# salute-developers/GigaAM

Hardware: AMD Instinct MI355X
Metric: RTFx v2_ctc batch32x20s (log-mel + encoder + greedy decode) (higher is better)
Workload: dtype f32 (GEMMs: 3-term split on fp16 MFMA, fp32 accumulate)

## Files before the change

### gigaam_amd/_lib.py

```python
from __future__ import annotations

import ctypes as C
import os
from typing import Optional

_HERE = os.path.dirname(os.path.abspath(__file__))
LIB_NAME = "libgigaam_hip.so"
LIB_PATH = os.path.join(_HERE, LIB_NAME)

SUBS_CONV2D, SUBS_CONV1D = 0, 1
ATT_ROTARY, ATT_REL_POS = 0, 1
NORM_BATCH, NORM_LAYER = 0, 1
HEAD_NONE, HEAD_CTC, HEAD_RNNT, HEAD_EMO = 0, 1, 2, 3
DTYPE_F32, DTYPE_F16, DTYPE_BF16, DTYPE_F64, DTYPE_I64 = 0, 1, 2, 3, 4
GEMM_F32, GEMM_F16X3, GEMM_F16 = 0, 1, 2
RS_U8, RS_I16, RS_I24, RS_I32, RS_F32, RS_MULAW, RS_ALAW = range(7)
RS_FORM_SINGLE, RS_FORM_TABLE, RS_FORM_ROWS = 0, 1, 2
PF_CLASSES = ["gemm", "conv2", "attn", "norm", "convmod", "stem", "frontend", "decode", "misc", "align_bt", "align_out"]


class GamConfig(C.Structure):
    _fields_ = [(n, C.c_int32) for n in (
        "sample_rate", "n_mels", "hop_length", "win_length", "n_fft", "center",
        "feat_in", "n_layers", "d_model", "subsampling", "subs_kernel_size", "subsampling_factor",
# ... 66 lines not shown
    "gam_op_ctc_confidence": (C.c_int, [_P, _P, _P, C.c_int, C.c_int64, C.c_int, _P, _P, _P, C.c_int, C.c_int, C.c_int, _P, _P, _P, _P]),
    "gam_op_ctc_confidence_long": (C.c_int, [_P, _P, C.c_int64, C.c_int, _P, _P, _P, C.c_int, C.c_int, C.c_int, C.c_int, _P, _P, _P, _P]),
    "gam_rnnt_confidence": (C.c_int, [_P, _P, _P, C.c_int, C.c_int64, _P, _P, _P, C.c_int, C.c_int, _P, _P, _P]),
    "gam_op_rnnt_confidence": (C.c_int, [_P, _P, _P, C.c_int, C.c_int64, _P, _P, _P, C.c_int, C.c_int, _P, _P, _P]),
    "gam_emo_probs": (C.c_int, [_P, _P, _P, C.c_int, C.c_int64, _P, _P]),
    "gam_rnnt_predict": (C.c_int, [_P, _P, _P, _P, C.c_int, _P, _P, _P, _P]),
    "gam_rnnt_joint": (C.c_int, [_P, _P, _P, C.c_int, C.c_int, C.c_int, _P, _P]),
    "gam_set_gemm_mode": (C.c_int, [_P, C.c_int]),
    "gam_get_gemm_mode": (C.c_int, [_P]),
    "gam_set_rnnt_cluster": (C.c_int, [_P, C.c_int]),
    "gam_get_rnnt_cluster": (C.c_int, [_P]),
    "gam_rnnt_cluster_plan_info": (C.c_int, [C.c_int] * 8 + [C.POINTER(C.c_int32)]),
    "gam_rnnt_last_decode": (C.c_int, [_P, C.POINTER(C.c_int32)]),
    "gam_debug_buffer_hash": (C.c_int, [_P, C.c_int, C.POINTER(C.c_uint64), C.POINTER(C.c_int64)]),
    "gam_range_flag": (C.c_int, [_P, C.POINTER(C.c_int), _P]),
    "gam_range_flag_fetch": (C.c_int, [_P, _P, _P]),
    "gam_op_gemm": (C.c_int, [_P, _P, _P, _P, _P, C.c_int, C.c_int, C.c_int, C.c_int, _P]),
    "gam_op_gemm_ex": (C.c_int, [_P, _P, _P, _P, _P, C.c_float, _P, C.c_int, C.c_int, C.c_int, C.c_int, _P]),
    "gam_op_attention": (C.c_int, [_P, _P, _P, _P, _P, _P, C.c_int, C.c_int, C.c_int, _P]),
    "gam_op_attention_ex": (C.c_int, [_P, _P, _P, _P, C.c_int64, _P, _P, _P, C.c_int, C.c_int, C.c_int, C.c_int, _P, _P, _P, _P]),
    "gam_op_layernorm": (C.c_int, [_P, C.POINTER(GamLnOp), _P]),
    "gam_op_convmod": (C.c_int, [_P, _P, _P, _P, _P, _P, _P, _P, _P, C.c_int, C.c_int, C.c_int, C.c_int, C.c_int, C.c_int, C.c_int, _P]),
    "gam_tune_sp": (C.c_int, [C.c_int, C.c_int, C.c_int]),
    "gam_plan_sp": (C.c_int, [C.c_int, C.c_int, C.c_int, C.c_int, C.POINTER(C.c_int), C.POINTER(C.c_int), C.POINTER(C.c_int)]),
    "gam_plan_sp_ex": (C.c_int, [C.c_int, C.c_int, C.c_int, C.c_int, C.POINTER(C.c_int), C.POINTER(C.c_int), C.POINTER(C.c_int), C.POINTER(C.c_int)]),
    "gam_tune_sp_stages": (C.c_int, [C.c_int]),
    "gam_resample_plan": (C.c_int, [C.c_int, C.c_int, C.POINTER(C.c_int), C.POINTER(C.c_int), C.POINTER(C.c_int)]),
    "gam_resample_tile": (C.c_int, [C.c_int, C.c_int, C.POINTER(C.c_int), C.POINTER(C.c_int)]),
    "gam_resample_table": (C.c_int, [C.c_int, C.c_int, _P, _P]),
    "gam_resample_out_len": (C.c_int64, [C.c_int, C.c_int, C.c_int64]),
    "gam_op_resample": (C.c_int, [_P, C.c_int, C.c_int, C.c_int, _P, C.c_int, C.c_int64, C.c_int, C.c_int, _P, _P, _P, C.c_int64, _P, _P]),
    "gam_profile_enable": (C.c_int, [_P, C.c_int]),
    "gam_profile_pause": (C.c_int, [_P, C.c_int]),
    "gam_profile_read": (C.c_int, [_P, C.c_int, C.POINTER(C.c_double), C.POINTER(C.c_int64), C.POINTER(C.c_double)]),
    "gam_profile_read_bytes": (C.c_int, [_P, C.c_int, C.POINTER(C.c_double)]),
    "gam_last_error": (C.c_char_p, [_P]),
    "gam_comm_unique_id": (C.c_int, [C.c_char_p]),
    "gam_comm_create": (C.c_int, [C.c_char_p, C.c_int, C.c_int, C.c_int, C.POINTER(_P)]),
    "gam_comm_world": (C.c_int, [_P]),
    "gam_gather_ids": (C.c_int, [_P, _P, _P, _P, _P, C.c_int, C.c_int, _P, _P, _P, _P, _P]),
    "gam_comm_last_error": (C.c_char_p, [_P]),
    "gam_comm_destroy": (None, [_P]),
}

_lib: Optional[C.CDLL] = None

# ... 25 lines not shown
```

### gigaam_amd/csrc/gam_api.hip

```cpp
#include <hip/hip_runtime.h>

#include <algorithm>
#include <cmath>
#include <cstdarg>
#include <cstdio>
#include <cstring>
#include <map>
#include <string>
#include <vector>

#include "../../include/gigaam_hip.h"
#include "gam_align.h"
#include "gam_align_long.h"
#include "gam_kws.h"
#include "gam_attn.h"
#include "gam_beam.h"
#include "gam_beam_stream.h"
#include "gam_rnnt_beam.h"
#include "gam_attn16.h"
#include "gam_comm.h"
#include "gam_common.h"
#include "gam_convmod.h"
#include "gam_decode.h"
#include "gam_rnnt_align.h"
// ... 410 lines not shown

GamGemmArgs gemm_args(const float* A, long lda, const float* W, const float* bias, float* C, long ldc, int M, int N, int K) {
  GamGemmArgs g;
  memset(&g, 0, sizeof g);
  g.A = A; g.W = W; g.bias = bias; g.C = C; g.R = nullptr;
  g.M = M; g.N = N; g.K = K; g.lda = lda; g.ldc = ldc; g.ldr = ldc; g.alpha = 1.0f;
  g.rpb = 1; g.fdiv = 1;
  return g;
}

int layernorm(gam_handle* h, hipStream_t s, GamLnArgs a, int mode, PendingReduce* pend = nullptr) {
  if (pend != nullptr && pend->part != nullptr) {
    const GamGemmArgs& g = pend->full;
    if (a.x == g.C && a.rows == g.M && a.d == g.N && g.ldc == g.N) {
      a.part = pend->part; a.nsplit = pend->nsplit; a.pbias = pend->bias; a.presid = pend->resid; a.palpha = pend->alpha;
      a.xstore = const_cast<float*>(a.x);
      pend->clear();
    } else if (int r = flush_pending(h, s, pend)) {
      return r;
    }
  }
  const double bytes = (double)a.rows * a.d * 4.0 * (mode == 0 ? 2.0 : 3.0);
  ProfScope ps(h, s, GAM_PF_NORM, bytes);
  hipError_t e = gam_launch_layernorm(a, mode, s);
  if (e != hipSuccess) return fail(h, -2, "layernorm launch: %s", hipGetErrorString(e));
  return 0;
}

int64_t half_up(int64_t l) { return l <= 0 ? 0 : (l + 1) / 2; }

struct DecodeScope {
  gam_handle* h;
  hipStream_t s;
  DecodeScope(gam_handle* h_, hipStream_t s_) : h(h_), s(s_) {
    if (h->dec_evt == nullptr && hipEventCreateWithFlags(&h->dec_evt, hipEventDisableTiming) != hipSuccess) { h->dec_evt = nullptr; (void)hipGetLastError(); }
    if (h->dec_evt != nullptr && h->dec_evt_set && h->dec_stream != s) (void)hipStreamWaitEvent(s, h->dec_evt, 0);
  }
  ~DecodeScope() {
    if (h->dec_evt != nullptr && hipEventRecord(h->dec_evt, s) == hipSuccess) { h->dec_stream = s; h->dec_evt_set = true; }
  }
};

#define GAM_DECODE_ENTRY(h, stream)      \
  hipStream_t s = (hipStream_t)(stream); \
  if (!(h)) return -1;                   \
  HIPCHK(h, hipSetDevice((h)->device));  \
  DecodeScope ds(h, s)
// ... 2252 lines not shown
    return fail(h, -1, "layernorm: store format %d / %d outside 0..2", o.split1, o.split2);
  if (!o.out1 || !o.w1 || !o.b1) return fail(h, -1, "layernorm: out1 / w1 / b1 are mandatory");
  if (!o.part && !o.x) return fail(h, -1, "layernorm: x is mandatory without part");
  if (o.part && o.mode != 2 && !o.xstore) return fail(h, -1, "layernorm: part without xstore");
  if (o.mode != 0 && !o.out2) return fail(h, -1, "layernorm: mode %d needs out2", o.mode);
  if (o.mode == 2 && (!o.w2 || !o.b2)) return fail(h, -1, "layernorm: mode 2 needs w2 / b2");
  if (o.mode == 1) {
    if (!o.rcos || !o.rsin || o.rope_rows <= 0) return fail(h, -1, "layernorm: mode 1 needs rcos / rsin of rope_rows > 0 rows");
    if (o.dk <= 0) return fail(h, -1, "layernorm: mode 1 needs dk > 0");
    if (!o.row_t && o.ta <= 0) return fail(h, -1, "layernorm: mode 1 needs row_t or ta > 0");
  }
  auto al16 = [](const void* p) { return (reinterpret_cast<uintptr_t>(p) & 15) == 0; };
  if (!al16(o.x) || !al16(o.out1) || !al16(o.out2) || !al16(o.w1) || !al16(o.b1) || !al16(o.w2) || !al16(o.b2) || !al16(o.rcos) ||
      !al16(o.rsin) || !al16(o.part) || !al16(o.pbias) || !al16(o.presid) || !al16(o.xstore))
    return fail(h, -1, "layernorm: operands must be 16-byte aligned");
  HIPCHK(h, hipSetDevice(h->device));
  GamLnArgs a;
  memset(&a, 0, sizeof a);
  a.x = o.x; a.out1 = o.out1; a.out2 = o.out2; a.w1 = o.w1; a.b1 = o.b1; a.w2 = o.w2; a.b2 = o.b2;
  a.rcos = o.rcos; a.rsin = o.rsin; a.rows = o.rows; a.d = o.d; a.ta = o.ta; a.dk = o.dk; a.eps = o.eps;
  a.split1 = o.split1; a.split2 = o.split2; a.rs = o.rs; a.rope_rows = o.rope_rows;
  a.part = o.part; a.nsplit = o.nsplit; a.pbias = o.pbias; a.presid = o.presid; a.palpha = o.palpha; a.xstore = o.xstore;
  a.row_t = o.row_t;
  hipError_t e = gam_launch_layernorm(a, o.mode, (hipStream_t)stream);
  if (e != hipSuccess)
    return fail(h, -2, "layernorm launch (mode %d, rows %d, d %d, dk %d, split %d/%d, nsplit %d): %s", o.mode, o.rows, o.d, o.dk,
                o.split1, o.split2, o.part ? o.nsplit : 0, hipGetErrorString(e));
  return 0;
}

int gam_op_convmod(gam_handle* h, const float* u, float* z, const float* dw_w, const float* dw_b, const float* n_scale,
                   const float* n_shift, const int32_t* lens, const int32_t* cu, int B, int Ta, int Tv, int d, int ks, int layer_norm,
                   int z_split, void* stream) {
  if (!h) return -1;
  if (!h->finalized) return fail(h, -1, "gam_op_convmod before gam_finalize");
  if (!u || !z || !dw_w || !dw_b || !n_scale || !n_shift || !lens) return fail(h, -1, "conv module: null operand");
  if (B <= 0 || Ta <= 0 || Tv <= 0 || d <= 0) return fail(h, -1, "conv module: bad shape B %d Ta %d Tv %d d %d", B, Ta, Tv, d);
  if (cu == nullptr && Tv > Ta) return fail(h, -1, "conv module: Tv %d > Ta %d in the padded layout", Tv, Ta);
  if (z_split < 0 || z_split > 2) return fail(h, -1, "conv module: store format %d outside 0..2", z_split);
  if (z_split && d % 32 != 0) return fail(h, -1, "conv module: a split-fp16 z needs d %% 32 == 0 (d = %d)", d);
  auto al16 = [](const void* p) { return (reinterpret_cast<uintptr_t>(p) & 15) == 0; };
  if (d % 4 == 0 && (!al16(u) || !al16(z) || !al16(dw_b) || !al16(n_scale) || !al16(n_shift)))
    return fail(h, -1, "conv module: operands must be 16-byte aligned");
  HIPCHK(h, hipSetDevice(h->device));
  hipError_t e = launch_convmod(h, (hipStream_t)stream, u, z, dw_w, dw_b, n_scale, n_shift, lens, cu, B, Ta, Tv, d, ks, layer_norm != 0, z_split);
  if (e != hipSuccess) return fail(h, -2, "conv-module launch (k=%d, d=%d, %s): %s", ks, d, layer_norm ? "LayerNorm" : "BatchNorm", hipGetErrorString(e));
  return 0;
// ... 67 lines not shown
int gam_range_flag_fetch(gam_handle* h, int32_t* flag_dev, void* stream) {
  if (!h || !flag_dev) return -1;
  if (!h->finalized) return fail(h, -1, "gam_range_flag_fetch before gam_finalize");
  HIPCHK(h, hipSetDevice(h->device));
  hipStream_t s = (hipStream_t)stream;
  HIPCHK(h, hipMemcpyAsync(flag_dev, h->range_flag, sizeof(int), hipMemcpyDeviceToDevice, s));
  HIPCHK(h, hipMemsetAsync(h->range_flag, 0, sizeof(int), s));
  return 0;
}

int gam_plan_sp(int M, int N, int K, int n_cu, int* mt, int* nw, int* splitk) {
  if (M <= 0 || N <= 0 || K <= 0 || K % 32 != 0 || !mt || !nw || !splitk) return -1;
  const GamSpPlan p = gam_gemm_sp_plan(M, N, K, 0, n_cu > 0 ? n_cu : 256);
  *mt = p.mt; *nw = p.nw; *splitk = p.s;
  return 0;
}

int gam_tune_sp(int mt, int nw, int splitk) {
  GamSpForce& f = gam_sp_force();
  f.mt = mt; f.nw = nw; f.s = splitk;
  return 0;
}

int gam_tune_sp_stages(int stages) {
  if (stages != 0 && stages != 2 && stages != 3) return -1;
  gam_sp_force().ns = stages;
  return 0;
}

int gam_plan_sp_ex(int M, int N, int K, int n_cu, int* mt, int* nw, int* splitk, int* stages) {
  if (M <= 0 || N <= 0 || K <= 0 || K % 32 != 0 || !mt || !nw || !splitk || !stages) return -1;
  const GamSpPlan p = gam_gemm_sp_plan(M, N, K, 0, n_cu > 0 ? n_cu : 256);
  *mt = p.mt; *nw = p.nw; *splitk = p.s; *stages = p.ns;
  return 0;
}

int gam_resample_plan(int rate_in, int rate_out, int* up, int* down, int* taps) {
  GamRsPlan p;
  const int rc = gam_rs_plan(rate_in, rate_out, &p);
  if (rc != 0) return rc;
  if (up) *up = (int)p.N;
  if (down) *down = (int)p.O;
  if (taps) *taps = p.K;
  return 0;
}

// ... 68 lines not shown
```

### gigaam_amd/csrc/gam_norm.h

```cpp
#pragma once
#include "gam_common.h"

#define GAM_LN_MAXJ 4
#define GAM_LN_EARLY_ROWS 1024

struct GamLnArgs {
  const float* x;
  float* out1;
  float* out2;
  const float* w1; const float* b1;
  const float* w2; const float* b2;
  const float* rcos; const float* rsin;
  int rows, d, ta, dk;
  float eps;
  int split1, split2;
  float* rs;
  int rope_rows;
  const float* part;
  int nsplit;
  const float* pbias;
  const float* presid;
  float palpha;
  float* xstore;
  const int* row_t;
};

__device__ __forceinline__ float gam_ln_rowmax(const float4 (&v)[GAM_LN_MAXJ], int d, int lane) {
  float m = 0.f;
#pragma unroll
  for (int j = 0; j < GAM_LN_MAXJ; ++j)
    if ((j * 64 + lane) * 4 < d) m = fmaxf(fmaxf(m, fmaxf(fabsf(v[j].x), fabsf(v[j].y))), fmaxf(fabsf(v[j].z), fabsf(v[j].w)));
  return gam_wave_max(m);
}

struct GamLnWB { float4 w[GAM_LN_MAXJ], b[GAM_LN_MAXJ]; };

__device__ __forceinline__ void gam_ln_load_wb(GamLnWB& p, const float* w, const float* b, int d, int lane) {
#pragma unroll
  for (int j = 0; j < GAM_LN_MAXJ; ++j) {
    const int c = (j * 64 + lane) * 4;
    p.w[j] = c < d ? *reinterpret_cast<const float4*>(w + c) : make_float4(0.f, 0.f, 0.f, 0.f);
    p.b[j] = c < d ? *reinterpret_cast<const float4*>(b + c) : make_float4(0.f, 0.f, 0.f, 0.f);
  }
}

template <bool PRE>
__device__ __forceinline__ void gam_ln_row(float4 (&v)[GAM_LN_MAXJ], int d, int lane, float eps, const GamLnWB& p,
                                           const float* w, const float* b) {
  float s = 0.f;
#pragma unroll
  for (int j = 0; j < GAM_LN_MAXJ; ++j)
    if ((j * 64 + lane) * 4 < d) s += (v[j].x + v[j].y) + (v[j].z + v[j].w);
  const float mean = gam_wave_sum(s) / (float)d;
  float q = 0.f;
#pragma unroll
  for (int j = 0; j < GAM_LN_MAXJ; ++j)
    if ((j * 64 + lane) * 4 < d) {
      const float a0 = v[j].x - mean, a1 = v[j].y - mean, a2 = v[j].z - mean, a3 = v[j].w - mean;
      q += (a0 * a0 + a1 * a1) + (a2 * a2 + a3 * a3);
    }
  const float rstd = 1.0f / sqrtf(gam_wave_sum(q) / (float)d + eps);
#pragma unroll
  for (int j = 0; j < GAM_LN_MAXJ; ++j) {
    const int c = (j * 64 + lane) * 4;
    if (c < d) {
      const float4 ww = PRE ? p.w[j] : *reinterpret_cast<const float4*>(w + c);
      const float4 bb = PRE ? p.b[j] : *reinterpret_cast<const float4*>(b + c);
      v[j].x = (v[j].x - mean) * rstd * ww.x + bb.x;
      v[j].y = (v[j].y - mean) * rstd * ww.y + bb.y;
      v[j].z = (v[j].z - mean) * rstd * ww.z + bb.z;
      v[j].w = (v[j].w - mean) * rstd * ww.w + bb.w;
    }
  }
}

template <int NS>
__device__ __forceinline__ void gam_ln_part_row(const GamLnArgs& a, int row, int lane, float4 (&v)[GAM_LN_MAXJ]) {
  const size_t slice = (size_t)a.rows * a.d;
  f32x4 sm[GAM_LN_MAXJ];
  float4 bb[GAM_LN_MAXJ], rr[GAM_LN_MAXJ];
#pragma unroll
  for (int j = 0; j < GAM_LN_MAXJ; ++j) {
    const int c0 = (j * 64 + lane) * 4, c = c0 < a.d ? c0 : 0;
    const float* p = a.part + (size_t)row * a.d + c;
    if constexpr (NS > 0) {
      sm[j] = gam_sum_slices_n<NS>(p, slice);
    } else {
      sm[j] = (f32x4){0.f, 0.f, 0.f, 0.f};
      for (int s_ = 0; s_ < a.nsplit; ++s_) sm[j] += *reinterpret_cast<const f32x4*>(p + s_ * slice);
    }
    bb[j] = *reinterpret_cast<const float4*>(a.pbias + c);
    rr[j] = *reinterpret_cast<const float4*>(a.presid + (size_t)row * a.d + c);
  }
#pragma unroll
  for (int j = 0; j < GAM_LN_MAXJ; ++j) {
    const bool in = (j * 64 + lane) * 4 < a.d;
    float4 acc = make_float4(sm[j].x + bb[j].x, sm[j].y + bb[j].y, sm[j].z + bb[j].z, sm[j].w + bb[j].w);
    acc.x = acc.x * a.palpha + rr[j].x; acc.y = acc.y * a.palpha + rr[j].y;
    acc.z = acc.z * a.palpha + rr[j].z; acc.w = acc.w * a.palpha + rr[j].w;
    v[j] = in ? acc : make_float4(0.f, 0.f, 0.f, 0.f);
  }
}

template <int MODE, bool PART = false, bool EARLY = false>
__global__ __launch_bounds__(256) void gam_layernorm_kernel(GamLnArgs a) {
  __shared__ float rowbuf[MODE == 1 ? 4 * GAM_LN_MAXJ * 256 : 4];
  const int lane = threadIdx.x & 63, wave = threadIdx.x >> 6;
  const int row_raw = blockIdx.x * 4 + wave;
  const bool live = row_raw < a.rows;
  const int row = live ? row_raw : a.rows - 1;
  const float* xr = a.x + (size_t)row * a.d;
  GamLnWB p1, p2;
  if (EARLY) gam_ln_load_wb(p1, a.w1, a.b1, a.d, lane);
  if (EARLY && MODE == 2) gam_ln_load_wb(p2, a.w2, a.b2, a.d, lane);
  float4 rc4[GAM_LN_MAXJ], rs4[GAM_LN_MAXJ];
  if (EARLY && MODE == 1) {
    int t = a.row_t != nullptr ? a.row_t[row] : row % a.ta;
    t = t < a.rope_rows ? t : a.rope_rows - 1;
    const int half = a.dk >> 1;
#pragma unroll
    for (int j = 0; j < GAM_LN_MAXJ; ++j) {
      const int c = (j * 64 + lane) * 4;
      const int i0 = c % a.dk, ib = i0 < half ? i0 : i0 - half;
      rc4[j] = c < a.d ? *reinterpret_cast<const float4*>(a.rcos + (size_t)t * half + ib) : make_float4(0.f, 0.f, 0.f, 0.f);
      rs4[j] = c < a.d ? *reinterpret_cast<const float4*>(a.rsin + (size_t)t * half + ib) : make_float4(0.f, 0.f, 0.f, 0.f);
    }
  }
  float4 v[GAM_LN_MAXJ];
  if constexpr (PART) {
    switch (a.nsplit) {
      case 2: gam_ln_part_row<2>(a, row, lane, v); break;
      case 3: gam_ln_part_row<3>(a, row, lane, v); break;
      case 4: gam_ln_part_row<4>(a, row, lane, v); break;
      case 6: gam_ln_part_row<6>(a, row, lane, v); break;
      case 8: gam_ln_part_row<8>(a, row, lane, v); break;
      default: gam_ln_part_row<0>(a, row, lane, v); break;
    }
    if (live && MODE != 2) {
#pragma unroll
      for (int j = 0; j < GAM_LN_MAXJ; ++j) {
        const int c = (j * 64 + lane) * 4;
        if (c < a.d) *reinterpret_cast<float4*>(a.xstore + (size_t)row * a.d + c) = v[j];
      }
    }
  } else {
#pragma unroll
    for (int j = 0; j < GAM_LN_MAXJ; ++j) {
      const int c = (j * 64 + lane) * 4;
      v[j] = c < a.d ? *reinterpret_cast<const float4*>(xr + c) : make_float4(0.f, 0.f, 0.f, 0.f);
    }
  }
  gam_ln_row<EARLY>(v, a.d, lane, a.eps, p1, a.w1, a.b1);
  float sc1 = 1.0f, sc2 = 1.0f;
  if (MODE != 2 && a.rs != nullptr) {
    float s_, inv_;
    gam_row_scale(gam_ln_rowmax(v, a.d, lane), s_, inv_);
    if (live && lane == 0) a.rs[row] = inv_;
    sc1 = s_;
    sc2 = s_;
  }
  if (live) {
#pragma unroll
    for (int j = 0; j < GAM_LN_MAXJ; ++j) {
      const int c = (j * 64 + lane) * 4;
      if (c < a.d) gam_store4(a.out1, (size_t)row * a.d, c, v[j].x * sc1, v[j].y * sc1, v[j].z * sc1, v[j].w * sc1, a.split1);
    }
  }
  if (MODE == 2) {
    gam_ln_row<EARLY>(v, a.d, lane, a.eps, p2, a.w2, a.b2);
    if (a.rs != nullptr) {
      float s_, inv_;
      gam_row_scale(gam_ln_rowmax(v, a.d, lane), s_, inv_);
      if (live && lane == 0) a.rs[row] = inv_;
      sc2 = s_;
    }
    if (live) {
#pragma unroll
      for (int j = 0; j < GAM_LN_MAXJ; ++j) {
        const int c = (j * 64 + lane) * 4;
        if (c < a.d) gam_store4(a.out2, (size_t)row * a.d, c, v[j].x * sc2, v[j].y * sc2, v[j].z * sc2, v[j].w * sc2, a.split2);
      }
    }
  }
  if (MODE == 1) {
    float* rb = rowbuf + wave * (GAM_LN_MAXJ * 256);
#pragma unroll
    for (int j = 0; j < GAM_LN_MAXJ; ++j) {
      const int c = (j * 64 + lane) * 4;
      if (c < a.d) *reinterpret_cast<float4*>(rb + c) = v[j];
    }
    __syncthreads();
    const int half = a.dk >> 1;
    int t = a.row_t != nullptr ? a.row_t[row] : row % a.ta;
    t = t < a.rope_rows ? t : a.rope_rows - 1;
#pragma unroll
    for (int j = 0; j < GAM_LN_MAXJ; ++j) {
      const int c = (j * 64 + lane) * 4;
      if (c < a.d) {
        float o[4];
        const int i0 = c % a.dk;
        const bool lo_half = i0 < half;
        const int po = lo_half ? half : -half;
        const float4 self4 = *reinterpret_cast<const float4*>(rb + c);
        const float4 oth4 = *reinterpret_cast<const float4*>(rb + c + po);
        const int ib = lo_half ? i0 : i0 - half;
        const float4 c4 = EARLY ? rc4[j] : *reinterpret_cast<const float4*>(a.rcos + (size_t)t * half + ib);
        const float4 s4 = EARLY ? rs4[j] : *reinterpret_cast<const float4*>(a.rsin + (size_t)t * half + ib);
        if (lo_half) {
          o[0] = self4.x * c4.x - oth4.x * s4.x; o[1] = self4.y * c4.y - oth4.y * s4.y;
          o[2] = self4.z * c4.z - oth4.z * s4.z; o[3] = self4.w * c4.w - oth4.w * s4.w;
        } else {
          o[0] = self4.x * c4.x + oth4.x * s4.x; o[1] = self4.y * c4.y + oth4.y * s4.y;
          o[2] = self4.z * c4.z + oth4.z * s4.z; o[3] = self4.w * c4.w + oth4.w * s4.w;
        }
        if (live) gam_store4(a.out2, (size_t)row * a.d, c, o[0] * sc2, o[1] * sc2, o[2] * sc2, o[3] * sc2, a.split2);
      }
    }
  }
}

static inline hipError_t gam_launch_layernorm(const GamLnArgs& a, int mode, hipStream_t s) {
  if (a.rows <= 0) return hipSuccess;
  if (a.d % 4 != 0 || a.d > GAM_LN_MAXJ * 256) return hipErrorInvalidValue;
  if ((a.split1 || a.split2) && a.d % 32 != 0) return hipErrorInvalidValue;
  if (mode == 1 && (a.dk % 8 != 0 || a.d % a.dk != 0)) return hipErrorInvalidValue;
  if (a.part != nullptr && (a.pbias == nullptr || a.presid == nullptr || a.nsplit < 1)) return hipErrorInvalidValue;
  const int grid = gam_cdiv(a.rows, 4);
  const bool early = a.rows <= GAM_LN_EARLY_ROWS;
#define GAM_LN_GO(MODE, PART, EARLY) hipLaunchKernelGGL((gam_layernorm_kernel<MODE, PART, EARLY>), dim3(grid), dim3(256), 0, s, a)
#define GAM_LN_MODE(PART, EARLY) \
  do { if (mode == 0) GAM_LN_GO(0, PART, EARLY); else if (mode == 1) GAM_LN_GO(1, PART, EARLY); else GAM_LN_GO(2, PART, EARLY); } while (0)
  if (a.part != nullptr) GAM_LN_MODE(true, true);
  else if (early) GAM_LN_MODE(false, true);
  else GAM_LN_MODE(false, false);
#undef GAM_LN_MODE
#undef GAM_LN_GO
  return hipGetLastError();
}
```

### gigaam_amd/engine.py

```python
from __future__ import annotations

import contextlib
import ctypes as C
import functools
import math
import os
import threading
from typing import Any, Callable, Dict, List, Mapping, Optional, Sequence, Tuple

import numpy as np
import torch
from torch import Tensor

from . import _lib
from ._lib import GamConfig, GigaAMHipError


def _get(cfg: Any, key: str, default: Any = None) -> Any:
    if cfg is None:
        return default
    if isinstance(cfg, Mapping):
        return cfg.get(key, default)
    return getattr(cfg, key, default)

# ... 1334 lines not shown
        if not (t.is_cuda and t.device == self.device and t.dtype == dtype and t.is_contiguous()):
            raise GigaAMHipError(f"{what}: {name} must be a contiguous {dtype} tensor on {self.device}")
        return t.data_ptr()

    def op_layernorm(self, mode: int, rows: int, d: int, x: Optional[Tensor], out1: Tensor, w1: Tensor, b1: Tensor, *,
                     out2: Optional[Tensor] = None, w2: Optional[Tensor] = None, b2: Optional[Tensor] = None, split1: int = 0,
                     split2: int = 0, rs: Optional[Tensor] = None, rcos: Optional[Tensor] = None, rsin: Optional[Tensor] = None,
                     dk: int = 0, ta: int = 0, rope_rows: Optional[int] = None, row_t: Optional[Tensor] = None,
                     part: Optional[Tensor] = None, nsplit: int = 0, pbias: Optional[Tensor] = None, presid: Optional[Tensor] = None,
                     palpha: float = 1.0, xstore: Optional[Tensor] = None, eps: float = 1e-5) -> None:
        what = "op_layernorm"
        op = _lib.GamLnOp()
        for name, t in (("x", x), ("out1", out1), ("out2", out2), ("w1", w1), ("b1", b1), ("w2", w2), ("b2", b2), ("rcos", rcos),
                        ("rsin", rsin), ("rs", rs), ("part", part), ("pbias", pbias), ("presid", presid), ("xstore", xstore)):
            setattr(op, name, self._op_ptr(what, name, t))
        op.row_t = self._op_ptr(what, "row_t", row_t, torch.int32)
        op.mode, op.rows, op.d, op.split1, op.split2, op.dk, op.ta, op.nsplit = mode, rows, d, split1, split2, dk, ta, nsplit
        op.rope_rows = (0 if rcos is None else rcos.shape[0]) if rope_rows is None else rope_rows
        op.eps, op.palpha = eps, palpha
        with torch.cuda.device(self.device):
            rc = self.lib.gam_op_layernorm(self._h, C.byref(op), self._stream())
        self._check(rc, "gam_op_layernorm")

    def op_convmod(self, u: Tensor, z: Tensor, dw_w: Tensor, dw_b: Tensor, n_scale: Tensor, n_shift: Tensor, lens: Tensor, B: int,
                   Ta: int, Tv: int, d: int, ks: int, layer_norm: bool, z_split: int = 0, cu: Optional[Tensor] = None) -> None:
        what = "op_convmod"
        ptrs = [self._op_ptr(what, n, t) for n, t in (("u", u), ("z", z), ("dw_w", dw_w), ("dw_b", dw_b), ("n_scale", n_scale),
                                                      ("n_shift", n_shift))]
        ptrs += [self._op_ptr(what, "lens", lens, torch.int32), self._op_ptr(what, "cu", cu, torch.int32)]
        with torch.cuda.device(self.device):
            rc = self.lib.gam_op_convmod(self._h, *ptrs, B, Ta, Tv, d, ks, int(bool(layer_norm)), z_split, self._stream())
        self._check(rc, "gam_op_convmod")

    def profile_enable(self, on=True) -> None:
        self._check(self.lib.gam_profile_enable(self._h, int(on)), "gam_profile_enable")

    def profile_level(self, on) -> None:
        self._check(self.lib.gam_profile_pause(self._h, int(on)), "gam_profile_pause")

    def profile_read(self) -> Dict[str, Dict[str, float]]:
        out = {}
        for i, name in enumerate(_lib.PF_CLASSES):
            ms, n, work = C.c_double(), C.c_int64(), C.c_double()
            self._check(self.lib.gam_profile_read(self._h, i, C.byref(ms), C.byref(n), C.byref(work)), "gam_profile_read")
            nbytes = C.c_double()
            self._check(self.lib.gam_profile_read_bytes(self._h, i, C.byref(nbytes)), "gam_profile_read_bytes")
# ... 3 lines not shown
```

### include/gigaam_hip.h

```cpp
#ifndef GIGAAM_HIP_H
#define GIGAAM_HIP_H

#include <stdint.h>

#ifdef __cplusplus
extern "C" {
#endif

#define GAM_ABI_VERSION 1

typedef struct gam_handle gam_handle;

enum { GAM_SUBS_CONV2D = 0, GAM_SUBS_CONV1D = 1 };
enum { GAM_ATT_ROTARY = 0, GAM_ATT_REL_POS = 1 };
enum { GAM_NORM_BATCH = 0, GAM_NORM_LAYER = 1 };
enum { GAM_HEAD_NONE = 0, GAM_HEAD_CTC = 1, GAM_HEAD_RNNT = 2, GAM_HEAD_EMO = 3 };
enum { GAM_DTYPE_F32 = 0, GAM_DTYPE_F16 = 1, GAM_DTYPE_BF16 = 2, GAM_DTYPE_F64 = 3, GAM_DTYPE_I64 = 4 };

typedef struct gam_config {
  int32_t sample_rate, n_mels, hop_length, win_length, n_fft, center;
  int32_t feat_in, n_layers, d_model, subsampling, subs_kernel_size, subsampling_factor;
  int32_t ff_expansion_factor, self_attention_model, n_heads, pos_emb_max_len;
  int32_t conv_norm_type, conv_kernel_size;
  int32_t head_type, num_classes, pred_hidden, pred_rnn_layers, joint_hidden;
// ... 160 lines not shown
                        const int32_t* lens, const int32_t* cu, int B, int Ta, int Tv, int H, const float* pbuf,
                        const float* pos_u, const float* pos_v, void* stream);

typedef struct gam_ln_op {
  const float* x;
  float* out1;
  float* out2;
  const float* w1;
  const float* b1;
  const float* w2;
  const float* b2;
  const float* rcos;
  const float* rsin;
  const int32_t* row_t;
  float* rs;
  const float* part;
  const float* pbias;
  const float* presid;
  float* xstore;
  int32_t mode, rows, d, split1, split2, dk, ta, rope_rows, nsplit;
  float eps, palpha;
} gam_ln_op;
int gam_op_layernorm(gam_handle* h, const gam_ln_op* op, void* stream);

int gam_op_convmod(gam_handle* h, const float* u, float* z, const float* dw_w, const float* dw_b, const float* n_scale,
                   const float* n_shift, const int32_t* lens, const int32_t* cu, int B, int Ta, int Tv, int d, int ks,
                   int layer_norm, int z_split, void* stream);

int gam_tune_sp(int mt, int nw, int splitk);
int gam_plan_sp(int M, int N, int K, int n_cu, int* mt, int* nw, int* splitk);
int gam_plan_sp_ex(int M, int N, int K, int n_cu, int* mt, int* nw, int* splitk, int* stages);
int gam_tune_sp_stages(int stages);

enum { GAM_RS_FMT_U8 = 0, GAM_RS_FMT_I16 = 1, GAM_RS_FMT_I24 = 2, GAM_RS_FMT_I32 = 3, GAM_RS_FMT_F32 = 4, GAM_RS_FMT_MULAW = 5,
       GAM_RS_FMT_ALAW = 6 };
int gam_resample_plan(int rate_in, int rate_out, int* up, int* down, int* taps);
int gam_resample_tile(int rate_in, int rate_out, int* tile, int* form);
int gam_resample_table(int rate_in, int rate_out, float* coeff, int32_t* first);
int64_t gam_resample_out_len(int rate_in, int rate_out, int64_t n_in);
int gam_op_resample(const void* src, int fmt, int channels, int channel, const int64_t* len_in, int B, int64_t frames, int rate_in,
                    int rate_out, const float* coeff, const int32_t* first, float* dst, int64_t L_out, int64_t* len_out, void* stream);

enum { GAM_PF_GEMM = 0, GAM_PF_CONV2 = 1, GAM_PF_ATTN = 2, GAM_PF_NORM = 3, GAM_PF_CONVMOD = 4,
       GAM_PF_STEM = 5, GAM_PF_FRONTEND = 6, GAM_PF_DECODE = 7, GAM_PF_MISC = 8,
       GAM_PF_ALIGN_BT = 9, GAM_PF_ALIGN_OUT = 10,
       GAM_PF_NCLASS = 11 };
// ... 23 lines not shown
```

Baseline: 21880.

## Replace large-row layernorm with persistent streaming kernel prefetching next row batch

For row counts above the early threshold without fused split-K partials, layernorm now runs a persistent grid-stride kernel sized to resident capacity. Each wave keeps weights and biases in registers once, double-buffers the next batch of rows (and RoPE cos/sin tables) while normalizing the current one, and uses DPP/permlane swap reductions. The goal is to hide global load latency and avoid reloading gamma/beta per row, at the cost of higher register pressure and new template instantiations. A tuning entry point lets callers force rows-in-flight and a workgroup cap.

Result: no change. 22000, median of 6 (+0.5%).

```diff
diff --git a/gigaam_amd/_lib.py b/gigaam_amd/_lib.py
--- a/gigaam_amd/_lib.py
+++ b/gigaam_amd/_lib.py
@@ -112,6 +112,7 @@
     "gam_op_layernorm": (C.c_int, [_P, C.POINTER(GamLnOp), _P]),
     "gam_op_convmod": (C.c_int, [_P, _P, _P, _P, _P, _P, _P, _P, _P, C.c_int, C.c_int, C.c_int, C.c_int, C.c_int, C.c_int, C.c_int, _P]),
     "gam_tune_sp": (C.c_int, [C.c_int, C.c_int, C.c_int]),
+    "gam_tune_ln": (C.c_int, [C.c_int, C.c_int]),
     "gam_plan_sp": (C.c_int, [C.c_int, C.c_int, C.c_int, C.c_int, C.POINTER(C.c_int), C.POINTER(C.c_int), C.POINTER(C.c_int)]),
     "gam_plan_sp_ex": (C.c_int, [C.c_int, C.c_int, C.c_int, C.c_int, C.POINTER(C.c_int), C.POINTER(C.c_int), C.POINTER(C.c_int), C.POINTER(C.c_int)]),
     "gam_tune_sp_stages": (C.c_int, [C.c_int]),
diff --git a/gigaam_amd/csrc/gam_api.hip b/gigaam_amd/csrc/gam_api.hip
--- a/gigaam_amd/csrc/gam_api.hip
+++ b/gigaam_amd/csrc/gam_api.hip
@@ -456,7 +456,7 @@
   }
   const double bytes = (double)a.rows * a.d * 4.0 * (mode == 0 ? 2.0 : 3.0);
   ProfScope ps(h, s, GAM_PF_NORM, bytes);
-  hipError_t e = gam_launch_layernorm(a, mode, s);
+  hipError_t e = gam_launch_layernorm(a, mode, s, h->ncu);
   if (e != hipSuccess) return fail(h, -2, "layernorm launch: %s", hipGetErrorString(e));
   return 0;
 }
@@ -2755,7 +2755,7 @@
   a.split1 = o.split1; a.split2 = o.split2; a.rs = o.rs; a.rope_rows = o.rope_rows;
   a.part = o.part; a.nsplit = o.nsplit; a.pbias = o.pbias; a.presid = o.presid; a.palpha = o.palpha; a.xstore = o.xstore;
   a.row_t = o.row_t;
-  hipError_t e = gam_launch_layernorm(a, o.mode, (hipStream_t)stream);
+  hipError_t e = gam_launch_layernorm(a, o.mode, (hipStream_t)stream, h->ncu);
   if (e != hipSuccess)
     return fail(h, -2, "layernorm launch (mode %d, rows %d, d %d, dk %d, split %d/%d, nsplit %d): %s", o.mode, o.rows, o.d, o.dk,
                 o.split1, o.split2, o.part ? o.nsplit : 0, hipGetErrorString(e));
@@ -2869,6 +2869,13 @@
   return 0;
 }
 
+int gam_tune_ln(int rows_in_flight, int max_workgroups) {
+  if ((rows_in_flight != 0 && rows_in_flight != 1 && rows_in_flight != 2 && rows_in_flight != 4) || max_workgroups < 0) return -1;
+  GamLnForce& f = gam_ln_force();
+  f.r = rows_in_flight; f.maxwg = max_workgroups;
+  return 0;
+}
+
 int gam_tune_sp_stages(int stages) {
   if (stages != 0 && stages != 2 && stages != 3) return -1;
   gam_sp_force().ns = stages;
diff --git a/gigaam_amd/csrc/gam_norm.h b/gigaam_amd/csrc/gam_norm.h
--- a/gigaam_amd/csrc/gam_norm.h
+++ b/gigaam_amd/csrc/gam_norm.h
@@ -44,9 +44,7 @@
   }
 }
 
-template <bool PRE>
-__device__ __forceinline__ void gam_ln_row(float4 (&v)[GAM_LN_MAXJ], int d, int lane, float eps, const GamLnWB& p,
-                                           const float* w, const float* b) {
+__device__ __forceinline__ void gam_ln_row(float4 (&v)[GAM_LN_MAXJ], int d, int lane, float eps, const GamLnWB& p) {
   float s = 0.f;
 #pragma unroll
   for (int j = 0; j < GAM_LN_MAXJ; ++j)
@@ -64,8 +62,7 @@
   for (int j = 0; j < GAM_LN_MAXJ; ++j) {
     const int c = (j * 64 + lane) * 4;
     if (c < d) {
-      const float4 ww = PRE ? p.w[j] : *reinterpret_cast<const float4*>(w + c);
-      const float4 bb = PRE ? p.b[j] : *reinterpret_cast<const float4*>(b + c);
+      const float4 ww = p.w[j], bb = p.b[j];
       v[j].x = (v[j].x - mean) * rstd * ww.x + bb.x;
       v[j].y = (v[j].y - mean) * rstd * ww.y + bb.y;
       v[j].z = (v[j].z - mean) * rstd * ww.z + bb.z;
@@ -102,7 +99,7 @@
   }
 }
 
-template <int MODE, bool PART = false, bool EARLY = false>
+template <int MODE, bool PART = false>
 __global__ __launch_bounds__(256) void gam_layernorm_kernel(GamLnArgs a) {
   __shared__ float rowbuf[MODE == 1 ? 4 * GAM_LN_MAXJ * 256 : 4];
   const int lane = threadIdx.x & 63, wave = threadIdx.x >> 6;
@@ -111,10 +108,10 @@
   const int row = live ? row_raw : a.rows - 1;
   const float* xr = a.x + (size_t)row * a.d;
   GamLnWB p1, p2;
-  if (EARLY) gam_ln_load_wb(p1, a.w1, a.b1, a.d, lane);
-  if (EARLY && MODE == 2) gam_ln_load_wb(p2, a.w2, a.b2, a.d, lane);
+  gam_ln_load_wb(p1, a.w1, a.b1, a.d, lane);
+  if (MODE == 2) gam_ln_load_wb(p2, a.w2, a.b2, a.d, lane);
   float4 rc4[GAM_LN_MAXJ], rs4[GAM_LN_MAXJ];
-  if (EARLY && MODE == 1) {
+  if (MODE == 1) {
     int t = a.row_t != nullptr ? a.row_t[row] : row % a.ta;
     t = t < a.rope_rows ? t : a.rope_rows - 1;
     const int half = a.dk >> 1;
@@ -150,7 +147,7 @@
       v[j] = c < a.d ? *reinterpret_cast<const float4*>(xr + c) : make_float4(0.f, 0.f, 0.f, 0.f);
     }
   }
-  gam_ln_row<EARLY>(v, a.d, lane, a.eps, p1, a.w1, a.b1);
+  gam_ln_row(v, a.d, lane, a.eps, p1);
   float sc1 = 1.0f, sc2 = 1.0f;
   if (MODE != 2 && a.rs != nullptr) {
     float s_, inv_;
@@ -167,7 +164,7 @@
     }
   }
   if (MODE == 2) {
-    gam_ln_row<EARLY>(v, a.d, lane, a.eps, p2, a.w2, a.b2);
+    gam_ln_row(v, a.d, lane, a.eps, p2);
     if (a.rs != nullptr) {
       float s_, inv_;
       gam_row_scale(gam_ln_rowmax(v, a.d, lane), s_, inv_);
@@ -191,8 +188,6 @@
     }
     __syncthreads();
     const int half = a.dk >> 1;
-    int t = a.row_t != nullptr ? a.row_t[row] : row % a.ta;
-    t = t < a.rope_rows ? t : a.rope_rows - 1;
 #pragma unroll
     for (int j = 0; j < GAM_LN_MAXJ; ++j) {
       const int c = (j * 64 + lane) * 4;
@@ -203,9 +198,7 @@
         const int po = lo_half ? half : -half;
         const float4 self4 = *reinterpret_cast<const float4*>(rb + c);
         const float4 oth4 = *reinterpret_cast<const float4*>(rb + c + po);
-        const int ib = lo_half ? i0 : i0 - half;
-        const float4 c4 = EARLY ? rc4[j] : *reinterpret_cast<const float4*>(a.rcos + (size_t)t * half + ib);
-        const float4 s4 = EARLY ? rs4[j] : *reinterpret_cast<const float4*>(a.rsin + (size_t)t * half + ib);
+        const float4 c4 = rc4[j], s4 = rs4[j];
         if (lo_half) {
           o[0] = self4.x * c4.x - oth4.x * s4.x; o[1] = self4.y * c4.y - oth4.y * s4.y;
           o[2] = self4.z * c4.z - oth4.z * s4.z; o[3] = self4.w * c4.w - oth4.w * s4.w;
@@ -219,21 +212,335 @@
   }
 }
 
-static inline hipError_t gam_launch_layernorm(const GamLnArgs& a, int mode, hipStream_t s) {
+
+struct GamLnAdd { __device__ __forceinline__ float operator()(float x, float y) const { return x + y; } };
+struct GamLnMax { __device__ __forceinline__ float operator()(float x, float y) const { return fmaxf(x, y); } };
+template <int CTRL>
+__device__ __forceinline__ float gam_ln_dpp(float v) {
+  return __int_as_float(__builtin_amdgcn_update_dpp(__float_as_int(v), __float_as_int(v), CTRL, 0xf, 0xf, false));
+}
+template <int O, class Op>
+__device__ __forceinline__ float gam_ln_xor_step(float v, Op op) {
+  if constexpr (O == 32) {
+    const auto r = __builtin_amdgcn_permlane32_swap(__float_as_uint(v), __float_as_uint(v), false, false);
+    return op(__uint_as_float(r[0]), __uint_as_float(r[1]));
+  } else if constexpr (O == 16) {
+    const auto r = __builtin_amdgcn_permlane16_swap(__float_as_uint(v), __float_as_uint(v), false, false);
+    return op(__uint_as_float(r[0]), __uint_as_float(r[1]));
+  } else if constexpr (O == 8) {
+    return op(v, gam_ln_dpp<0x128>(v));
+  } else if constexpr (O == 4) {
+    return op(v, gam_ln_dpp<0x1b>(gam_ln_dpp<0x141>(v)));
+  } else if constexpr (O == 2) {
+    return op(v, gam_ln_dpp<0x4e>(v));
+  } else {
+    return op(v, gam_ln_dpp<0xb1>(v));
+  }
+}
+template <int R, class Op>
+__device__ __forceinline__ void gam_ln_wave_reduce(float (&s)[R], Op op) {
+#pragma unroll
+  for (int r = 0; r < R; ++r) s[r] = gam_ln_xor_step<32>(s[r], op);
+#pragma unroll
+  for (int r = 0; r < R; ++r) s[r] = gam_ln_xor_step<16>(s[r], op);
+#pragma unroll
+  for (int r = 0; r < R; ++r) s[r] = gam_ln_xor_step<8>(s[r], op);
+#pragma unroll
+  for (int r = 0; r < R; ++r) s[r] = gam_ln_xor_step<4>(s[r], op);
+#pragma unroll
+  for (int r = 0; r < R; ++r) s[r] = gam_ln_xor_step<2>(s[r], op);
+#pragma unroll
+  for (int r = 0; r < R; ++r) s[r] = gam_ln_xor_step<1>(s[r], op);
+}
+
+template <int NJ> struct GamLnWBn { float4 w[NJ], b[NJ]; };
+template <int NJ>
+__device__ __forceinline__ void gam_ln_load_wbn(GamLnWBn<NJ>& p, const float* w, const float* b, int d, int lane) {
+#pragma unroll
+  for (int j = 0; j < NJ; ++j) {
+    const int c = (j * 64 + lane) * 4, cc = c < d ? c : 0;
+    p.w[j] = *reinterpret_cast<const float4*>(w + cc);
+    p.b[j] = *reinterpret_cast<const float4*>(b + cc);
+  }
+}
+
+template <int R, int NJ>
+__device__ __forceinline__ void gam_ln_rows(float4 (&v)[R][NJ], int d, int lane, float eps, const GamLnWBn<NJ>& p) {
+  float s[R], q[R], mean[R], rstd[R];
+#pragma unroll
+  for (int r = 0; r < R; ++r) {
+    s[r] = 0.f;
+#pragma unroll
+    for (int j = 0; j < NJ; ++j)
+      if ((j * 64 + lane) * 4 < d) s[r] += (v[r][j].x + v[r][j].y) + (v[r][j].z + v[r][j].w);
+  }
+  gam_ln_wave_reduce<R>(s, GamLnAdd());
+#pragma unroll
+  for (int r = 0; r < R; ++r) {
+    mean[r] = s[r] / (float)d;
+    q[r] = 0.f;
+#pragma unroll
+    for (int j = 0; j < NJ; ++j)
+      if ((j * 64 + lane) * 4 < d) {
+        const float a0 = v[r][j].x - mean[r], a1 = v[r][j].y - mean[r], a2 = v[r][j].z - mean[r], a3 = v[r][j].w - mean[r];
+        q[r] += (a0 * a0 + a1 * a1) + (a2 * a2 + a3 * a3);
+      }
+  }
+  gam_ln_wave_reduce<R>(q, GamLnAdd());
+#pragma unroll
+  for (int r = 0; r < R; ++r) {
+    rstd[r] = 1.0f / sqrtf(q[r] / (float)d + eps);
+#pragma unroll
+    for (int j = 0; j < NJ; ++j) {
+      if ((j * 64 + lane) * 4 < d) {
+        const float4 ww = p.w[j], bb = p.b[j];
+        v[r][j].x = (v[r][j].x - mean[r]) * rstd[r] * ww.x + bb.x;
+        v[r][j].y = (v[r][j].y - mean[r]) * rstd[r] * ww.y + bb.y;
+        v[r][j].z = (v[r][j].z - mean[r]) * rstd[r] * ww.z + bb.z;
+        v[r][j].w = (v[r][j].w - mean[r]) * rstd[r] * ww.w + bb.w;
+      }
+    }
+  }
+}
+
+template <int R, int NJ>
+__device__ __forceinline__ void gam_ln_rows_scale(const float4 (&v)[R][NJ], int d, int lane, const int (&row)[R], const bool (&live)[R],
+                                                  float* rs, float (&sc)[R]) {
+  float m[R];
+#pragma unroll
+  for (int r = 0; r < R; ++r) {
+    m[r] = 0.f;
+#pragma unroll
+    for (int j = 0; j < NJ; ++j)
+      if ((j * 64 + lane) * 4 < d)
+        m[r] = fmaxf(fmaxf(m[r], fmaxf(fabsf(v[r][j].x), fabsf(v[r][j].y))), fmaxf(fabsf(v[r][j].z), fabsf(v[r][j].w)));
+  }
+  gam_ln_wave_reduce<R>(m, GamLnMax());
+#pragma unroll
+  for (int r = 0; r < R; ++r) {
+    float inv_;
+    gam_row_scale(m[r], sc[r], inv_);
+    if (live[r] && lane == 0) rs[row[r]] = inv_;
+  }
+}
+
+template <int R, int NJ>
+__device__ __forceinline__ void gam_ln_rows_store(const float4 (&v)[R][NJ], int d, int lane, const int (&row)[R], const bool (&live)[R],
+                                                  float* out, const float (&sc)[R], int split) {
+#pragma unroll
+  for (int r = 0; r < R; ++r)
+    if (live[r]) {
+#pragma unroll
+      for (int j = 0; j < NJ; ++j) {
+        const int c = (j * 64 + lane) * 4;
+        if (c < d) gam_store4(out, (size_t)row[r] * d, c, v[r][j].x * sc[r], v[r][j].y * sc[r], v[r][j].z * sc[r], v[r][j].w * sc[r], split);
+      }
+    }
+}
+
+
+__device__ __forceinline__ void gam_ln_arrived(float4& x) { asm volatile("" : "+v"(x.x), "+v"(x.y), "+v"(x.z), "+v"(x.w)); }
+__device__ __forceinline__ int gam_ln_batch_row(const GamLnArgs& a, long base, int r) {
+  return base + r < a.rows ? (int)(base + r) : a.rows - 1;
+}
+template <int R, int NJ>
+__device__ __forceinline__ void gam_ln_rows_load(const GamLnArgs& a, long base, int lane, float4 (&v)[R][NJ]) {
+#pragma unroll
+  for (int r = 0; r < R; ++r) {
+    const float* xr = a.x + (size_t)gam_ln_batch_row(a, base, r) * a.d;
+#pragma unroll
+    for (int j = 0; j < NJ; ++j) {
+      const int c = (j * 64 + lane) * 4;
+      v[r][j] = *reinterpret_cast<const float4*>(xr + (c < a.d ? c : 0));
+    }
+  }
+}
+template <int R, bool PACKED>
+__device__ __forceinline__ void gam_ln_frames_load(const GamLnArgs& a, long base, int (&t)[R]) {
+#pragma unroll
+  for (int r = 0; r < R; ++r) {
+    const int row = gam_ln_batch_row(a, base, r);
+    t[r] = PACKED ? a.row_t[row] : row % a.ta;
+  }
+}
+template <int R, int NJ>
+__device__ __forceinline__ void gam_ln_rope_load(const GamLnArgs& a, const int (&t)[R], int lane, float4 (&rc4)[R][NJ], float4 (&rs4)[R][NJ]) {
+  const int half = a.dk >> 1;
+#pragma unroll
+  for (int r = 0; r < R; ++r) {
+    const int tc = t[r] < a.rope_rows ? t[r] : a.rope_rows - 1;
+#pragma unroll
+    for (int j = 0; j < NJ; ++j) {
+      const int c = (j * 64 + lane) * 4;
+      const int i0 = (c < a.d ? c : 0) % a.dk, ib = i0 < half ? i0 : i0 - half;
+      rc4[r][j] = *reinterpret_cast<const float4*>(a.rcos + (size_t)tc * half + ib);
+      rs4[r][j] = *reinterpret_cast<const float4*>(a.rsin + (size_t)tc * half + ib);
+    }
+  }
+}
+
+template <int MODE, int R, int NJ, bool PACKED>
+__device__ __forceinline__ void gam_ln_stream_batch(const GamLnArgs& a, long base, long stride, int lane, float* rb,
+                                                    const GamLnWBn<NJ>& p1, const GamLnWBn<NJ>& p2, float4 (&v)[R][NJ], float4 (&vn)[R][NJ],
+                                                    float4 (&rc4)[MODE == 1 ? R : 1][NJ], float4 (&rs4)[MODE == 1 ? R : 1][NJ],
+                                                    int (&tn)[MODE == 1 ? R : 1], int (&tnn)[MODE == 1 ? R : 1]) {
+  constexpr int RR = MODE == 1 ? R : 1;
+  gam_ln_rows_load<R, NJ>(a, base + stride, lane, vn);
+  if (MODE == 1) {
+    gam_ln_frames_load<RR, PACKED>(a, base + 2 * stride, tnn);
+#pragma unroll
+    for (int r = 0; r < RR; ++r) {
+#pragma unroll
+      for (int j = 0; j < NJ; ++j) { gam_ln_arrived(rc4[r][j]); gam_ln_arrived(rs4[r][j]); }
+      asm volatile("" : "+v"(tn[r]));
+    }
+  }
+  int row[R];
+  bool live[R];
+#pragma unroll
+  for (int r = 0; r < R; ++r) {
+    live[r] = base + r < a.rows;
+    row[r] = gam_ln_batch_row(a, base, r);
+  }
+
+  gam_ln_rows<R, NJ>(v, a.d, lane, a.eps, p1);
+  float sc1[R], sc2[R];
+#pragma unroll
+  for (int r = 0; r < R; ++r) sc1[r] = sc2[r] = 1.0f;
+  if (MODE != 2 && a.rs != nullptr) {
+    gam_ln_rows_scale<R, NJ>(v, a.d, lane, row, live, a.rs, sc1);
+#pragma unroll
+    for (int r = 0; r < R; ++r) sc2[r] = sc1[r];
+  }
+  gam_ln_rows_store<R, NJ>(v, a.d, lane, row, live, a.out1, sc1, a.split1);
+  if (MODE == 2) {
+    gam_ln_rows<R, NJ>(v, a.d, lane, a.eps, p2);
+    if (a.rs != nullptr) gam_ln_rows_scale<R, NJ>(v, a.d, lane, row, live, a.rs, sc2);
+    gam_ln_rows_store<R, NJ>(v, a.d, lane, row, live, a.out2, sc2, a.split2);
+  }
+  if (MODE == 1) {
+    const int half = a.dk >> 1;
+    float4 o4[RR][NJ];
+#pragma unroll
+    for (int r = 0; r < RR; ++r) {
+#pragma unroll
+      for (int j = 0; j < NJ; ++j) {
+        const int c = (j * 64 + lane) * 4;
+        if (c < a.d) *reinterpret_cast<float4*>(rb + c) = v[r][j];
+      }
+      __builtin_amdgcn_wave_barrier();
+#pragma unroll
+      for (int j = 0; j < NJ; ++j) {
+        const int c = (j * 64 + lane) * 4;
+        if (c < a.d) {
+          float o[4];
+          const int i0 = c % a.dk;
+          const bool lo_half = i0 < half;
+          const int po = lo_half ? half : -half;
+          const float4 self4 = v[r][j];
+          const float4 oth4 = *reinterpret_cast<const float4*>(rb + c + po);
+          const float4 c4 = rc4[r][j], s4 = rs4[r][j];
+          if (lo_half) {
+            o[0] = self4.x * c4.x - oth4.x * s4.x; o[1] = self4.y * c4.y - oth4.y * s4.y;
+            o[2] = self4.z * c4.z - oth4.z * s4.z; o[3] = self4.w * c4.w - oth4.w * s4.w;
+          } else {
+            o[0] = self4.x * c4.x + oth4.x * s4.x; o[1] = self4.y * c4.y + oth4.y * s4.y;
+            o[2] = self4.z * c4.z + oth4.z * s4.z; o[3] = self4.w * c4.w + oth4.w * s4.w;
+          }
+          o4[r][j] = make_float4(o[0] * sc2[r], o[1] * sc2[r], o[2] * sc2[r], o[3] * sc2[r]);
+        }
+      }
+      __builtin_amdgcn_wave_barrier();
+    }
+    gam_ln_rope_load<RR, NJ>(a, tn, lane, rc4, rs4);
+#pragma unroll
+    for (int r = 0; r < RR; ++r)
+      if (live[r]) {
+#pragma unroll
+        for (int j = 0; j < NJ; ++j) {
+          const int c = (j * 64 + lane) * 4;
+          if (c < a.d) gam_store4(a.out2, (size_t)row[r] * a.d, c, o4[r][j].x, o4[r][j].y, o4[r][j].z, o4[r][j].w, a.split2);
+        }
+      }
+  }
+}
+
+template <int MODE, int R, int NJ, bool PACKED = false>
+__global__ __launch_bounds__(256) void gam_layernorm_stream_kernel(GamLnArgs a) {
+  constexpr int RR = MODE == 1 ? R : 1;
+  __shared__ float rowbuf[MODE == 1 ? 4 * NJ * 256 : 4];
+  const int lane = threadIdx.x & 63, wave = __builtin_amdgcn_readfirstlane(threadIdx.x >> 6);
+  float* rb = rowbuf + (MODE == 1 ? wave * (NJ * 256) : 0);
+  const long stride = (long)gridDim.x * 4 * R;
+  long base = ((long)blockIdx.x * 4 + wave) * R;
+  if (base >= a.rows) return;
+  GamLnWBn<NJ> p1, p2;
+  gam_ln_load_wbn(p1, a.w1, a.b1, a.d, lane);
+  if (MODE == 2) gam_ln_load_wbn(p2, a.w2, a.b2, a.d, lane);
+  float4 va[R][NJ], vb[R][NJ], rc4[RR][NJ], rs4[RR][NJ];
+  int ta[RR], tb[RR];
+  gam_ln_rows_load<R, NJ>(a, base, lane, va);
+  if (MODE == 1) {
+    gam_ln_frames_load<RR, PACKED>(a, base, tb);
+    gam_ln_frames_load<RR, PACKED>(a, base + stride, ta);
+    gam_ln_rope_load<RR, NJ>(a, tb, lane, rc4, rs4);
+  }
+  for (;;) {
+    gam_ln_stream_batch<MODE, R, NJ, PACKED>(a, base, stride, lane, rb, p1, p2, va, vb, rc4, rs4, ta, tb);
+    base += stride;
+    if (base >= a.rows) break;
+    gam_ln_stream_batch<MODE, R, NJ, PACKED>(a, base, stride, lane, rb, p1, p2, vb, va, rc4, rs4, tb, ta);
+    base += stride;
+    if (base >= a.rows) break;
+  }
+}
+
+#define GAM_LN_STREAM_R 1
+struct GamLnForce { std::atomic<int> r{0}, maxwg{0}; };
+static inline GamLnForce& gam_ln_force() { static GamLnForce f; return f; }
+
+template <int MODE, int R, int NJ, bool PACKED = false>
+static inline void gam_ln_stream_go(const GamLnArgs& a, int ncu, int maxwg, hipStream_t s) {
+  static const int resident = [] {
+    int n = 0;
+    if (hipOccupancyMaxActiveBlocksPerMultiprocessor(&n, gam_layernorm_stream_kernel<MODE, R, NJ, PACKED>, 256, 0) != hipSuccess || n < 1) n = 1;
+    return n;
+  }();
+  const int units = gam_cdiv(a.rows, 4 * R);
+  long cap = (long)(ncu > 0 ? ncu : 256) * resident;
+  if (maxwg > 0 && maxwg < cap) cap = maxwg;
+  const int passes = gam_cdiv(units, cap);
+  const int grid = gam_cdiv(units, passes);
+  hipLaunchKernelGGL((gam_layernorm_stream_kernel<MODE, R, NJ, PACKED>), dim3(grid), dim3(256), 0, s, a);
+}
+
+static inline hipError_t gam_launch_layernorm(const GamLnArgs& a, int mode, hipStream_t s, int ncu = 256) {
   if (a.rows <= 0) return hipSuccess;
   if (a.d % 4 != 0 || a.d > GAM_LN_MAXJ * 256) return hipErrorInvalidValue;
   if ((a.split1 || a.split2) && a.d % 32 != 0) return hipErrorInvalidValue;
   if (mode == 1 && (a.dk % 8 != 0 || a.d % a.dk != 0)) return hipErrorInvalidValue;
   if (a.part != nullptr && (a.pbias == nullptr || a.presid == nullptr || a.nsplit < 1)) return hipErrorInvalidValue;
-  const int grid = gam_cdiv(a.rows, 4);
-  const bool early = a.rows <= GAM_LN_EARLY_ROWS;
-#define GAM_LN_GO(MODE, PART, EARLY) hipLaunchKernelGGL((gam_layernorm_kernel<MODE, PART, EARLY>), dim3(grid), dim3(256), 0, s, a)
-#define GAM_LN_MODE(PART, EARLY) \
-  do { if (mode == 0) GAM_LN_GO(0, PART, EARLY); else if (mode == 1) GAM_LN_GO(1, PART, EARLY); else GAM_LN_GO(2, PART, EARLY); } while (0)
-  if (a.part != nullptr) GAM_LN_MODE(true, true);
-  else if (early) GAM_LN_MODE(false, true);
-  else GAM_LN_MODE(false, false);
+  if (a.part != nullptr || a.rows <= GAM_LN_EARLY_ROWS) {
+    const int grid = gam_cdiv(a.rows, 4);
+#define GAM_LN_GO(MODE, PART) hipLaunchKernelGGL((gam_layernorm_kernel<MODE, PART>), dim3(grid), dim3(256), 0, s, a)
+#define GAM_LN_MODE(PART) do { if (mode == 0) GAM_LN_GO(0, PART); else if (mode == 1) GAM_LN_GO(1, PART); else GAM_LN_GO(2, PART); } while (0)
+    if (a.part != nullptr) GAM_LN_MODE(true);
+    else GAM_LN_MODE(false);
 #undef GAM_LN_MODE
 #undef GAM_LN_GO
+    return hipGetLastError();
+  }
+  const int fr = gam_ln_force().r.load(), maxwg = gam_ln_force().maxwg.load();
+  const int r = fr > 0 ? fr : GAM_LN_STREAM_R;
+#define GAM_LN_NJ(MODE, R, PACKED) \
+  do { if (a.d <= 768) gam_ln_stream_go<MODE, R, 3, PACKED>(a, ncu, maxwg, s); else gam_ln_stream_go<MODE, R, GAM_LN_MAXJ, PACKED>(a, ncu, maxwg, s); } while (0)
+#define GAM_LN_R(MODE, PACKED) \
+  do { if (r == 1) GAM_LN_NJ(MODE, 1, PACKED); else if (r == 2) GAM_LN_NJ(MODE, 2, PACKED); else GAM_LN_NJ(MODE, 4, PACKED); } while (0)
+  if (mode == 0) GAM_LN_R(0, false);
+  else if (mode == 2) GAM_LN_R(2, false);
+  else if (a.row_t != nullptr) GAM_LN_R(1, true);
+  else GAM_LN_R(1, false);
+#undef GAM_LN_R
+#undef GAM_LN_NJ
   return hipGetLastError();
 }
diff --git a/gigaam_amd/engine.py b/gigaam_amd/engine.py
--- a/gigaam_amd/engine.py
+++ b/gigaam_amd/engine.py
@@ -1380,6 +1380,10 @@
             rc = self.lib.gam_op_layernorm(self._h, C.byref(op), self._stream())
         self._check(rc, "gam_op_layernorm")
 
+    def tune_layernorm(self, rows_in_flight: int = 0, max_workgroups: int = 0) -> None:
+        if self.lib.gam_tune_ln(int(rows_in_flight), int(max_workgroups)) != 0:
+            raise GigaAMHipError(f"gam_tune_ln: rows_in_flight={rows_in_flight} must be 0, 1, 2 or 4, max_workgroups={max_workgroups} >= 0")
+
     def op_convmod(self, u: Tensor, z: Tensor, dw_w: Tensor, dw_b: Tensor, n_scale: Tensor, n_shift: Tensor, lens: Tensor, B: int,
                    Ta: int, Tv: int, d: int, ks: int, layer_norm: bool, z_split: int = 0, cu: Optional[Tensor] = None) -> None:
         what = "op_convmod"
diff --git a/include/gigaam_hip.h b/include/gigaam_hip.h
--- a/include/gigaam_hip.h
+++ b/include/gigaam_hip.h
@@ -206,6 +206,7 @@
   float eps, palpha;
 } gam_ln_op;
 int gam_op_layernorm(gam_handle* h, const gam_ln_op* op, void* stream);
+int gam_tune_ln(int rows_in_flight, int max_workgroups);
 
 int gam_op_convmod(gam_handle* h, const float* u, float* z, const float* dw_w, const float* dw_b, const float* n_scale,
                    const float* n_shift, const int32_t* lens, const int32_t* cu, int B, int Ta, int Tv, int d, int ks,
```
